# wing02/MyLdpcCppApi

Measured on AMD Instinct MI355X. Metric: decoded Mbit/s (info bits), DVB-S2 N=64800 rate-1/2, 50 iters, higher is better.
Workload: dtype f32; 1 GPU; DVB-S2-profile (64800,32400) rate-1/2 (seeded IRA table with the standard's structure, E=226799), batch 4096 frames per GPU, 50 iterations, sum-product fp32 (probability domain), all-zero codeword + AWGN sigma=0.95 (no frame converges), early termination on, inputs resident in HBM; global_batch=4096, frames_per_gpu=4096, algo=sp, frames_per_launch=4096, parallelism=frames sharded over 1 GPU(s), all-gather of decoded bytes, frames_converged=0

## Files before the change

myldpccppapi_amd/csrc/engine_flood.hip:

```cpp
#include <hip/hip_runtime.h>

#include <algorithm>
#include <map>
#include <vector>

#include "flood_round.hpp"
#include "flood_handover.hpp"
#include "crc_term_kernels.hpp"
#include "decoder.hpp"
#include "graph.hpp"

using ldpc::set_error;

namespace {

using ldpc::DevBuf;
using ldpc::RowClass;
using ldpc::ColClass;
using ldpc::ClassGroup;
using ldpc::kIdleFat;
using ldpc::dispatch_v;
using ldpc::span_begin;
using ldpc::span_end;
using ldpc::kVarBuckets;
using ldpc::kCheckBuckets;
using ldpc::kVarBucketLo;
using ldpc::kVarBucketHi;
using ldpc::kCheckBucketLo;
using ldpc::kCheckBucketHi;

template <int V>
__global__ void summary_kernel(const int32_t *iters, const uint64_t *done, const uint64_t *fail,
                               int64_t frames, int32_t freeze, int32_t *summary)
{
    constexpr int F = 64 * V;
    const int64_t f = (int64_t)blockIdx.x * blockDim.x + threadIdx.x;
    if (f >= frames) return;
    const int64_t tile = f / F;
    const int fi = (int)(f % F);
    const int l = fi / V, v = fi % V;
    atomicMax(&summary[0], iters[f]);
    const uint64_t ok = freeze ? done[tile * V + v] : ~fail[tile * V + v];
    if ((ok >> l) & 1ull) atomicAdd(&summary[1], 1);
}

static inline dim3 flood_grid(const ldpc_decoder *d, unsigned blocks, unsigned tiles, int32_t *tiles_first, bool linked = false)
{
    const bool want = d->tune.tiles_first == 1 || (d->tune.tiles_first == 0 && linked);
    *tiles_first = (blocks <= 65535u && want) ? 1 : 0;
    return *tiles_first ? dim3(tiles, blocks) : dim3(blocks, tiles);
}

static ldpc::CheckArgs check_args(const ldpc_decoder *d, const ldpc::TailRef &tr, int rows_per_wave, bool from_chan,
                                  const int32_t *e0 = nullptr, int n_rows = 0, int degree = 0)
{
    ldpc::CheckArgs a{d->flood.Q.p, d->flood.R.p, e0, d->done.p, d->E, n_rows, rows_per_wave, degree, d->ms_scale, tr};
    a.ms_offset = d->ms_offset;
    a.qpos = d->flood.qpos.p;
// ... 1 lines not shown
    return a;
}

template <int V> int run_flooding(ldpc_decoder *d, const float *llr_dev, int64_t frames,
                                  uint8_t *out_dev, int64_t out_bytes, int32_t *iters_dev,
                                  hipStream_t s, int start_round = 1);

template <int V> int enqueue_check_phase(ldpc_decoder *d, hipStream_t s, int tiles, int64_t frames, int it, int max_iter,
                                         bool fat, const ldpc::TailRef &tr)
{
    using namespace ldpc;
    const int64_t msz = d->flood.msg_size;
    const bool from_chan = it == 1 && d->flood.first_round_from_chan;
    for (auto &rc : d->flood.row_classes) {
        if (!rc.linked) continue;
        LDPC_HIP_TRY(span_begin(d, s, 4, rc.degree,
                           (2 * msz * rc.degree * rc.count + msz * 5 * rc.linked + 2 * msz * d->flood.extra_edges) * frames,
                           msz * ((int64_t)rc.degree * rc.count + rc.linked +
                                  ((int64_t)rc.degree * rc.count - 2 * rc.linked) +
                                  (it < max_iter ? 2 * rc.linked : 0) + 2 * d->flood.extra_edges) * frames));
        CheckArgs a = check_args(d, tr, d->flood.link_rpw, false, rc.e0.p, rc.count, rc.degree);
        LinkArgs lk{rc.link_col.p, rc.link_pos.p, d->flood.chan.p, d->flood.Q.p, d->hard.p, d->N,
                    (it < max_iter) ? 1 : 0, d->tm.tap_iter ? 1 : 0, d->flood.extra_e0.p, d->flood.extra_deg.p, d->flood.n_extra, 0,
                    rc.n_big, rc.small_rows};
        const int variant = (d->flood.link_form == 2 && !d->flood.fns.link_half[rc.degree]) ? 1 : d->flood.link_form;
        const int waves = link_chunk_count(d->flood.link_rpw, rc.n_big, rc.small_rows, rc.count) * (variant == 1 ? V : variant == 2 ? V / 2 : 1);
        lk.link_blocks = (waves + kWavesPerBlock - 1) / kWavesPerBlock;
        const dim3 grid = flood_grid(d, lk.link_blocks + (d->flood.n_extra + kWavesPerBlock - 1) / kWavesPerBlock, tiles, &a.tiles_first, true);
        (variant == 2 ? d->flood.fns.link_half : variant == 1 ? (d->flood.link_deep ? d->flood.fns.link_deep : d->flood.fns.link_narrow) : d->flood.fns.link)
            [rc.degree]<<<grid, kBlock, 0, s>>>(a, lk);
        LDPC_HIP_TRY(span_end(d, s));
    }
    for (auto &g : d->flood.check_groups) {
        int64_t edges = 0;
        for (int i : g.members) edges += (int64_t)d->flood.row_classes[i].degree * d->flood.row_classes[i].count;
        LDPC_HIP_TRY(span_begin(d, s, 5, g.hi, 2 * msz * edges * frames, -1, g.lo));
        CheckArgs a = check_args(d, tr, (d->tune.rows_per_wave ? d->tune.rows_per_wave : 2) * (fat ? kIdleFat : 1), from_chan);
        const dim3 grid = flood_grid(d, fat ? g.blocks_fat : g.blocks, tiles, &a.tiles_first);
        d->flood.fns.check_group[g.bucket]<<<grid, kBlock, 0, s>>>(a, fat ? g.table_fat.p : g.table.p, (int)g.members.size());
        LDPC_HIP_TRY(span_end(d, s));
    }
    for (int ci : d->flood.check_solo) {
        RowClass &rc = d->flood.row_classes[ci];
        LDPC_HIP_TRY(span_begin(d, s, 0, rc.degree, 2 * msz * rc.degree * rc.count * frames));
        const int slotk = rc.degree <= d->flood.fns.max_check_unrolled ? rc.degree : 0;
// ... 117 lines not shown
        } else {
            (void)hipGetLastError();
        }
    }
    const int idle_after = (freeze && !resume && !d->tm.tap_iter && d->cfg.poll_interval == 0) ? d->flood.idle_after : 0;
    const bool use_tail = d->flood.tail_enabled && freeze && !resume && !d->tm.tap_iter && tiles >= 4 * d->flood.TO;
    const TailRef tr{use_tail ? d->flood.tail_state.p : nullptr, d->T, d->flood.TO};
    TailArgs ta{};
    if (use_tail) {
        LDPC_HIP_TRY(hipMemsetAsync(d->flood.tail_state.p, 0, 4 * sizeof(int32_t), s));
        LDPC_HIP_TRY(hipMemsetAsync(d->flood.running.p, 0, d->flood.running.n * sizeof(int32_t), s));
        ta = TailArgs{d->flood.tail_state.p, d->flood.tail_map.p, d->flood.running.p, d->done.p, d->iters.p, d->flood.Q.p, d->flood.chan.p, d->hard.p,
                      d->E, frames, d->N, tiles, d->T, d->flood.TO * F, std::min(d->flood.compact_threshold, d->flood.TO * F), 0, max_iter};
    }

    bool q_less = d->cfg.algo == LDPC_ALGO_MS && !resume && !d->tm.tap_iter && max_iter > 1 && d->flood.n_extra == 0;
    for (auto &rc : d->flood.row_classes) if (rc.linked) q_less = false;
    for (int ci : d->flood.check_solo) if (d->flood.row_classes[ci].degree > d->flood.fns.max_check_unrolled) q_less = false;
    d->flood.first_round_from_chan = q_less;
    if (!resume) {
        LDPC_HIP_TRY(span_begin(d, s, 3));
        InitArgs a{llr_dev, d->flood.chan.p, q_less ? nullptr : d->flood.Q.p, d->hard.p, d->col_ptr.p, d->flood.col_qedge.p,
                   d->E, frames, d->N, d->cfg.llr_scale};
        dim3 grid((d->N + kInitCols - 1) / kInitCols, tiles);
        d->flood.fns.init<<<grid, kBlock, 0, s>>>(a);
        StateArgs st{d->done.p, nullptr, d->iters.p, nullptr, frames, 0, max_iter, freeze ? 1 : 0};
        state_kernel<V><<<use_tail ? d->flood.TA : tiles, 64, 0, s>>>(st);
        LDPC_HIP_TRY(span_end(d, s));
    }

    int launched = start_round - 1;
    bool poll_dense = false;
    for (int it = start_round; it <= rounds; ++it) {
        const bool fat = idle_after > 0 && it > idle_after;
        {
            const int rcp = enqueue_check_phase<V>(d, s, tiles, frames, it, max_iter, fat, tr);
            if (rcp) return rcp;
        }
        {
            const int rcv = enqueue_var_phase<V>(d, s, tiles, frames, it, max_iter, fat, tr);
            if (rcv) return rcv;
        }
        launched = it;
        if (freeze || it == rounds) {
            LDPC_HIP_TRY(span_begin(d, s, 3));
            uint64_t *fw = d->failw.p + (size_t)it * slot;
            const int rbk = (d->M + kBlock - 1) / kBlock;
            SyndromeArgs sa{d->row_ptr.p, d->edge_col.p, d->hard.p, fw, d->done.p, d->M, d->N,
                            d->flood.syn_xcd ? tiles : 0, rbk, tr};
            dim3 sgrid = d->flood.syn_xcd ? dim3(8 * rbk * ((tiles + 7) / 8)) : dim3(rbk, tiles);
            syndrome_kernel<V><<<sgrid, kBlock, 0, s>>>(sa);
            if (d->cfg.crc_kind) {
                CrcTermArgs ca{d->hard.p, fw, d->done.p, d->crc_w.p, d->summary.p + 3, d->N, d->cfg.crc_bits, tr};
                crc_term_kernel<V><<<dim3((unsigned)tiles, V), 64 * crc_term_waves(d->cfg.crc_bits), 0, s>>>(ca);
            }
            StateArgs st{d->done.p, fw, d->iters.p, nullptr, frames, it, max_iter, 1, tr, use_tail ? d->flood.running.p : nullptr,
                         d->summary.p + 2};
            const bool poll = freeze && it < rounds && d->cfg.poll_interval > 0 && !d->host.suppress_poll &&
                              ((it % d->cfg.poll_interval) == 0 || poll_dense);
            if (poll) {
                LDPC_HIP_TRY(hipMemsetAsync(d->active.p, 0, sizeof(int32_t), s));
                st.active = d->active.p;
            }
            state_kernel<V><<<tiles, 64, 0, s>>>(st);
// ... 290 lines not shown

template <int V> int time_check_phase(ldpc_decoder *d, float *ms_out)
{
    hipStream_t s = d->stream.s;
    LDPC_HIP_TRY(hipMemsetAsync(d->flood.Q.p, 0, d->flood.Q.n, s));
    LDPC_HIP_TRY(hipMemsetAsync(d->flood.chan.p, 0, d->flood.chan.n, s));
    LDPC_HIP_TRY(hipMemsetAsync(d->done.p, 0, d->done.n * sizeof(uint64_t), s));
    ldpc::Event ev[2];
    LDPC_HIP_TRY(ev[0].create());
    LDPC_HIP_TRY(ev[1].create());
    float best = 1e30f;
    hipError_t err = hipSuccess;
    int rc = LDPC_OK;
    for (int rep = 0; rep < 4 && err == hipSuccess && rc == LDPC_OK; ++rep) {
        err = hipEventRecord(ev[0].e, s);
        rc = enqueue_check_phase<V>(d, s, d->T, (int64_t)d->T * d->F, 1, d->cfg.max_iter, false, ldpc::TailRef{nullptr, 0, 0});
        if (rc == LDPC_OK)
            rc = enqueue_var_phase<V>(d, s, d->T, (int64_t)d->T * d->F, 1, d->cfg.max_iter, false, ldpc::TailRef{nullptr, 0, 0});
        if (err == hipSuccess) err = hipEventRecord(ev[1].e, s);
        if (err == hipSuccess) err = hipEventSynchronize(ev[1].e);
        float ms = 0;
        if (err == hipSuccess) err = hipEventElapsedTime(&ms, ev[0].e, ev[1].e);
        if (err == hipSuccess && rep > 0 && ms < best) best = ms;
    }
    if (rc) return rc;
    if (err != hipSuccess) return set_error(LDPC_ERR_HIP, "placement search: %s", hipGetErrorString(err));
    *ms_out = best;
    return LDPC_OK;
}

template <int V> int placement_search(ldpc_decoder *d, size_t TF)
{
    const size_t bq = TF * (size_t)d->E * d->flood.msg_size, bc = TF * d->N * d->flood.msg_size;
// ... 62 lines not shown
```

myldpccppapi_amd/csrc/flood_check.hpp:

```cpp
#pragma once

#include "flood_common.hpp"

namespace ldpc {

template <int D, int V>
__device__ __forceinline__ void check_sp(const float (&x)[D][V], float (&out)[D][V])
{
#pragma unroll
    for (int v = 0; v < V; ++v) {
        if (D == 1) { out[0][v] = 1.0f; continue; }
        {
            float p = x[1][v];
#pragma unroll
            for (int j = 2; j < D; ++j) p *= x[j][v];
            out[0][v] = p;
        }
        float pre = x[0][v];
#pragma unroll
        for (int k = 1; k < D; ++k) {
            float p = pre;
#pragma unroll
            for (int j = k + 1; j < D; ++j) p *= x[j][v];
            out[k][v] = p;
// ... 70 lines not shown
    const int tile = tile_select<V>(a.tail, a.done, gp.row);
    if (tile < 0) return;
    const int wave = gp.block * kWavesPerBlock + wave_id_in_block();
    const int sub = wave % SUB;
    const int r_begin = (wave / SUB) * a.rows_per_wave;
    const int r_end = min(r_begin + a.rows_per_wave, a.n_rows);
    const unsigned lane_off = (unsigned)sub * 64 * W + (unsigned)lane * W;
    const T *Qu = static_cast<const T *>(a.Q) + (size_t)tile * (size_t)a.E * F;
    T *Rt = static_cast<T *>(a.R) + (size_t)tile * (size_t)a.E * F + lane_off;

    const T *Ct = (ALGO != kAlgoSP && a.first_chan)
                      ? static_cast<const T *>(a.first_chan) + (size_t)tile * (size_t)a.N * F + lane_off : nullptr;
    check_rows<ALGO, D, V, W, T>(Qu, lane_off, Rt, a.cls_e0, r_begin, r_end, Ct, a.edge_col, a.qpos, ms_corr_of(a));
}

template <int ALGO, int V, typename T>
__device__ __forceinline__ void check_row_generic(const T *Qu, unsigned lane_off, T *Rt, int e0, int D,
                                                  const int32_t *__restrict__ qpos, const MsCorr &c)
{
    constexpr size_t F = 64 * V;
    if (ALGO != kAlgoSP) {
        float m1[V], m2[V];
        int idx[V];
        unsigned par[V];
#pragma unroll
        for (int v = 0; v < V; ++v) { m1[v] = 1000.0f; m2[v] = 1000.0f; idx[v] = -1; par[v] = 0; }
        for (int j = 0; j < D; ++j) {
            float xj[V];
            vload<V>(xj, Qu + (size_t)edge_slot(qpos, e0 + j) * F + lane_off);
#pragma unroll
            for (int v = 0; v < V; ++v) {
                const float m = __builtin_fabsf(xj[v]);
                par[v] ^= (xj[v] < 0.0f) ? 1u : 0u;
                if (m < m1[v]) { m2[v] = m1[v]; m1[v] = m; idx[v] = j; }
                else if (m < m2[v]) { m2[v] = m; }
            }
        }
        if (ALGO == kAlgoMSC) {
#pragma unroll
            for (int v = 0; v < V; ++v) { m1[v] = ms_corr<T>(m1[v], c); m2[v] = ms_corr<T>(m2[v], c); }
        }
        for (int k = 0; k < D; ++k) {
            float xk[V], o[V];
            vload<V>(xk, Qu + (size_t)edge_slot(qpos, e0 + k) * F + lane_off);
#pragma unroll
            for (int v = 0; v < V; ++v) {
                const float b = (k == idx[v]) ? m2[v] : m1[v];
                const unsigned sg = par[v] ^ ((xk[v] < 0.0f) ? 1u : 0u);
                o[v] = sg ? -b : b;
            }
            vstore<V>(Rt + (size_t)(e0 + k) * F, o);
        }
        return;
    }
    for (int k = 0; k < D; ++k) {
        float o[V];
        float p[V];
#pragma unroll
        for (int v = 0; v < V; ++v) p[v] = 1.0f;
        for (int j = 0; j < D; ++j) {
            if (j == k) continue;
            float xj[V];
            vload<V>(xj, Qu + (size_t)edge_slot(qpos, e0 + j) * F + lane_off);
#pragma unroll
            for (int v = 0; v < V; ++v) p[v] *= xj[v];
        }
#pragma unroll
        for (int v = 0; v < V; ++v) o[v] = p[v];
        vstore<V>(Rt + (size_t)(e0 + k) * F, o);
    }
}

template <int ALGO, int V, typename T>
__global__ __launch_bounds__(kBlock) void check_kernel_generic(const CheckArgs a)
{
    constexpr size_t F = 64 * V;
    const int lane = threadIdx.x & 63;
    const GridPos gp = grid_pos(a.tiles_first);
// ... 51 lines not shown
```

myldpccppapi_amd/csrc/flood_common.hpp:

```cpp
#pragma once

#include <hip/hip_runtime.h>
#include <stdint.h>

namespace ldpc {

constexpr int kAlgoSP = 0;
constexpr int kAlgoMS = 1;
constexpr int kAlgoMSC = 2;
constexpr int kCompactCapacity = 512;
constexpr int kLastCapacity = 64;
constexpr int kBlock = 256;
constexpr int kWavesPerBlock = 4;
constexpr int kMaxUnrolledDegree = 16;
constexpr int kMaxUnrolledCheckDegreeMS = 32;

#ifndef LDPC_NT_LOAD
#define LDPC_NT_LOAD 1
#endif
#ifndef LDPC_NT_STORE
#define LDPC_NT_STORE 1
#endif
typedef float vf2 __attribute__((ext_vector_type(2)));
typedef float vf4 __attribute__((ext_vector_type(4)));
// ... 117 lines not shown
    const int32_t *__restrict__ qpos = nullptr;
};

template <int D> __device__ __forceinline__ void row_slots(const int32_t *__restrict__ qpos, int e0, int lane, int (&slot)[D])
{
    static_assert(D <= 64, "one lane per edge");
    const int mine = qpos[e0 + (lane < D ? lane : D - 1)];
#pragma unroll
    for (int k = 0; k < D; ++k) slot[k] = __builtin_amdgcn_readlane(mine, k);
}
__device__ __forceinline__ int edge_slot(const int32_t *__restrict__ qpos, int e)
{
    return __builtin_amdgcn_readfirstlane(qpos[e]);
}

struct GridPos { int row, block; };
__device__ __forceinline__ GridPos grid_pos(int tiles_first)
{
    return tiles_first ? GridPos{(int)blockIdx.x, (int)blockIdx.y} : GridPos{(int)blockIdx.y, (int)blockIdx.x};
}

struct MsCorr {
    float scale, offset;
};
template <typename T> __device__ __forceinline__ float ms_corr(float m, const MsCorr &c)
{
    const float r = fmaxf(m - c.offset, 0.0f) * c.scale;
    return sizeof(T) == 2 ? (float)(hf)r : r;
}

// ... 53 lines not shown
```

myldpccppapi_amd/csrc/flood_link.hpp:

```cpp
#pragma once

#include "flood_check.hpp"
#include "flood_var.hpp"

namespace ldpc {

struct LinkArgs {
    const int32_t *__restrict__ link_col;
    const int32_t *__restrict__ link_pos;
    const void *__restrict__ chan;
    void *Qw;
    uint64_t *hard;
    int32_t N;
    int32_t write_q;
    int32_t store_all;
    const int32_t *__restrict__ extra_e0;
    const int32_t *__restrict__ extra_deg;
    int32_t n_extra;
    int32_t link_blocks;
    int32_t n_big, small_rows;
};

__host__ __device__ inline void link_chunk_rows(int c, int rows_per_wave, int n_big, int small_rows, int n_rows,
                                               int *rb, int *re)
{
    int b, e;
    if (c < n_big) { b = c * rows_per_wave; e = b + rows_per_wave; }
    else { b = n_big * rows_per_wave + (c - n_big) * small_rows; e = b + small_rows; }
    *rb = b < n_rows ? b : n_rows;
    *re = e < n_rows ? e : n_rows;
}
__host__ __device__ inline int link_chunk_count(int rows_per_wave, int n_big, int small_rows, int n_rows)
{
    const int rest = n_rows - n_big * rows_per_wave;
    return n_big + (rest > 0 ? (rest + small_rows - 1) / small_rows : 0);
}

template <int ALGO, int V, typename T>
__device__ __forceinline__ void link_extra_rows(const CheckArgs &a, const LinkArgs &g, int tile, int block)
{
    constexpr size_t F = 64 * V;
    const int lane = threadIdx.x & 63;
    const int w = (block - g.link_blocks) * kWavesPerBlock + wave_id_in_block();
    if (w >= g.n_extra) return;
    const T *Qu = static_cast<const T *>(a.Q) + (size_t)tile * (size_t)a.E * F;
    T *Rt = static_cast<T *>(a.R) + (size_t)tile * (size_t)a.E * F + (size_t)lane * V;
    check_row_generic<ALGO, V, T>(Qu, (unsigned)lane * V, Rt, g.extra_e0[w], g.extra_deg[w], a.qpos, ms_corr_of(a));
}

#ifdef LDPC_LINK_WIDE_WAVES
#define LDPC_LINK_WIDE_ATTR __attribute__((amdgpu_waves_per_eu(LDPC_LINK_WIDE_WAVES, LDPC_LINK_WIDE_WAVES)))
#else
#define LDPC_LINK_WIDE_ATTR
#endif
template <int ALGO, int D, int V, typename T>
__global__ __launch_bounds__(kBlock) LDPC_LINK_WIDE_ATTR void check_link_kernel(const CheckArgs a, const LinkArgs g)
{
    constexpr size_t F = 64 * V;
    const int lane = threadIdx.x & 63;
    const GridPos gp = grid_pos(a.tiles_first);
    const int tile = tile_select<V>(a.tail, a.done, gp.row);
    if (tile < 0) return;
    if (gp.block >= g.link_blocks) { link_extra_rows<ALGO, V, T>(a, g, tile, gp.block); return; }
    const int wave = gp.block * kWavesPerBlock + wave_id_in_block();
    int r_begin, r_end;
    link_chunk_rows(wave, a.rows_per_wave, g.n_big, g.small_rows, a.n_rows, &r_begin, &r_end);
    const size_t lane_off = (size_t)lane * V;
    const unsigned lane_q = (unsigned)lane * V;
    const T *Qt = static_cast<const T *>(a.Q) + (size_t)tile * (size_t)a.E * F;
    T *Qwt = static_cast<T *>(g.Qw) + (size_t)tile * (size_t)a.E * F;
    T *Rt = static_cast<T *>(a.R) + (size_t)tile * (size_t)a.E * F + lane_off;
    const T *chan_t = static_cast<const T *>(g.chan) + (size_t)tile * (size_t)g.N * F + lane_off;
    uint64_t *hard_t = g.hard + (size_t)tile * (size_t)g.N * V;
    uint64_t frozen[V];
#pragma unroll
    for (int v = 0; v < V; ++v) frozen[v] = a.done[(size_t)tile * V + v];

    int pend_col = -1, pend_edge = 0, pend_kb = 0;
    float pend_r[V];
#pragma unroll
    for (int v = 0; v < V; ++v) pend_r[v] = 0.0f;

    float x[D][V];
    int qc[D], qn[D];
#pragma unroll
    for (int k = 0; k < D; ++k) qc[k] = qn[k] = 0;
    if (r_begin < r_end) {
        row_slots<D>(a.qpos, a.cls_e0[r_begin], lane, qc);
#pragma unroll
        for (int k = 0; k < D; ++k) vload<V>(x[k], Qt + (size_t)qc[k] * F + lane_q);
    }
    for (int r = r_begin; r < r_end; ++r) {
        const int e0 = a.cls_e0[r];
        const int next_col = (r + 1 < r_end) ? g.link_col[r] : -1;
        const int pos = g.link_pos[r];
        const int ka = next_col >= 0 ? (pos & 255) : -1;
        const int kb = pend_col >= 0 ? pend_kb : -1;
        if (r + 1 < r_end) row_slots<D>(a.qpos, a.cls_e0[r + 1], lane, qn);
        float ch[V];
        uint64_t old_w[V];
        if (pend_col >= 0) {
            vload<V>(ch, chan_t + (size_t)pend_col * F);
#pragma unroll
            for (int v = 0; v < V; ++v) old_w[v] = hard_t[(size_t)pend_col * V + v];
        }
        float out[D][V];
        check_node<ALGO, D, V, T>(x, out, ms_corr_of(a));
        if (r + 1 < r_end) {
#pragma unroll
            for (int k = 0; k < D; ++k) vload<V>(x[k], Qt + (size_t)qn[k] * F + lane_q);
        }
#pragma unroll
        for (int k = 0; k < D; ++k)
            if ((k != ka && k != kb) || g.store_all) vstore<V>(Rt + (size_t)(e0 + k) * F, out[k]);

        if (pend_col >= 0) {
            float rr[2][V], q[2][V];
#pragma unroll
            for (int v = 0; v < V; ++v) {
                rr[0][v] = pend_r[v];
                float t = out[0][v];
#pragma unroll
                for (int k = 1; k < D; ++k) t = (k == kb) ? out[k][v] : t;
                rr[1][v] = t;
            }
// ... 38 lines not shown
            for (int k = 1; k < D; ++k) pend_edge = (k == ka) ? qc[k] : pend_edge;
            pend_kb = (pos >> 8) & 255;
#pragma unroll
            for (int v = 0; v < V; ++v) {
                float t = out[0][v];
#pragma unroll
                for (int k = 1; k < D; ++k) t = (k == ka) ? out[k][v] : t;
                pend_r[v] = t;
            }
        }
#pragma unroll
        for (int k = 0; k < D; ++k) qc[k] = qn[k];
    }
}

template <int ALGO, int D, int V, typename T, int W = 1>
__global__ __launch_bounds__(kBlock) void check_link_narrow_kernel(const CheckArgs a, const LinkArgs g)
{
    constexpr size_t F = 64 * V;
    constexpr int SUBS = V / W;
    constexpr int FB = 64 / SUBS;
    const int lane = threadIdx.x & 63;
    const GridPos gp = grid_pos(a.tiles_first);
    const int tile = tile_select<V>(a.tail, a.done, gp.row);
    if (tile < 0) return;
    if (gp.block >= g.link_blocks) { link_extra_rows<ALGO, V, T>(a, g, tile, gp.block); return; }
    const int wave = gp.block * kWavesPerBlock + wave_id_in_block();
    const int sub = wave % SUBS;
    int r_begin, r_end;
    link_chunk_rows(wave / SUBS, a.rows_per_wave, g.n_big, g.small_rows, a.n_rows, &r_begin, &r_end);
    const size_t lane_off = (size_t)sub * 64 * W + (size_t)lane * W;
    const unsigned lane_q = (unsigned)lane_off;
    const T *Qt = static_cast<const T *>(a.Q) + (size_t)tile * (size_t)a.E * F;
    T *Qwt = static_cast<T *>(g.Qw) + (size_t)tile * (size_t)a.E * F;
    T *Rt = static_cast<T *>(a.R) + (size_t)tile * (size_t)a.E * F + lane_off;
    const T *chan_t = static_cast<const T *>(g.chan) + (size_t)tile * (size_t)g.N * F + lane_off;
    uint8_t *hard_b = reinterpret_cast<uint8_t *>(g.hard + (size_t)tile * (size_t)g.N * V) + (size_t)sub * (FB / 8);
    const uint64_t frozen_field = (a.done[(size_t)tile * V + (lane < V ? lane : 0)] >> (sub * FB)) &
                                  (FB == 64 ? ~0ull : ((1ull << (FB & 63)) - 1ull));

    auto load_field = [&](int col, int word) -> uint64_t {
// ... 1 lines not shown
        if (FB == 64) return *reinterpret_cast<const uint64_t *>(p);
        if (FB == 32) return *reinterpret_cast<const uint32_t *>(p);
        return *reinterpret_cast<const uint16_t *>(p);
    };

    int pend_col = -1, pend_edge = 0, pend_kb = 0;
    float pend_r[W];
#pragma unroll
    for (int w = 0; w < W; ++w) pend_r[w] = 0.0f;
    float x[D][W];
    int qc[D], qn[D];
#pragma unroll
    for (int k = 0; k < D; ++k) qc[k] = qn[k] = 0;
    if (r_begin < r_end) {
        row_slots<D>(a.qpos, a.cls_e0[r_begin], lane, qc);
#pragma unroll
        for (int k = 0; k < D; ++k) vload<W>(x[k], Qt + (size_t)qc[k] * F + lane_q);
    }
    for (int r = r_begin; r < r_end; ++r) {
        const int e0 = a.cls_e0[r];
        const int next_col = (r + 1 < r_end) ? g.link_col[r] : -1;
        const int pos = g.link_pos[r];
        const int ka = next_col >= 0 ? (pos & 255) : -1;
        const int kb = pend_col >= 0 ? pend_kb : -1;
        if (r + 1 < r_end) row_slots<D>(a.qpos, a.cls_e0[r + 1], lane, qn);
        float ch[W];
        uint64_t old_mine[W];
#pragma unroll
        for (int w = 0; w < W; ++w) { ch[w] = 0.0f; old_mine[w] = 0; }
        if (pend_col >= 0) {
            vload<W>(ch, chan_t + (size_t)pend_col * F);
#pragma unroll
            for (int w = 0; w < W; ++w) old_mine[w] = load_field(pend_col, (W * lane + w) % V);
        }
        float out[D][W];
        check_node<ALGO, D, W, T>(x, out, ms_corr_of(a));
        if (r + 1 < r_end) {
#pragma unroll
            for (int k = 0; k < D; ++k) vload<W>(x[k], Qt + (size_t)qn[k] * F + lane_q);
        }
#pragma unroll
        for (int k = 0; k < D; ++k)
            if ((k != ka && k != kb) || g.store_all) vstore<W>(Rt + (size_t)(e0 + k) * F, out[k]);

        if (pend_col >= 0) {
            float rr[2][W], q[2][W];
#pragma unroll
            for (int w = 0; w < W; ++w) {
                rr[0][w] = pend_r[w];
                float t = out[0][w];
#pragma unroll
                for (int k = 1; k < D; ++k) t = (k == kb) ? out[k][w] : t;
                rr[1][w] = t;
            }
// ... 177 lines not shown
```

myldpccppapi_amd/csrc/flood_round.hpp:

```cpp
#pragma once

#include "flood_common.hpp"
#include "ldpc_expf.h"

namespace ldpc {

struct InitArgs {
    const float *__restrict__ llr;
    void *__restrict__ chan;
    void *__restrict__ Q;
    uint64_t *__restrict__ hard;
    const int32_t *__restrict__ col_ptr;
    const int32_t *__restrict__ col_edge;
    int64_t E;
    int64_t frames;
    int32_t N;
    float llr_scale;
};

constexpr int kInitCols = 32;

template <int ALGO, int V, typename T>
__global__ __launch_bounds__(kBlock) void init_kernel(const InitArgs a)
{
// ... 29 lines not shown
            patch[c * LD + f] = y;
        }
    }
    __syncthreads();
    const int lane = threadIdx.x & 63;
    for (int c = threadIdx.x >> 6; c < kInitCols; c += kWavesPerBlock) {
        const int n = n0 + c;
        if (n >= a.N) break;
        float ch[V], q[V];
#pragma unroll
        for (int v = 0; v < V; ++v) {
            const float y = patch[c * LD + lane * V + v];
            if (ALGO == kAlgoSP) {
                const float t = ldpc_expf(a.llr_scale * y);
                ch[v] = t;
                q[v] = t / (1.0f + t) - 1.0f / (1.0f + t);
            } else {
                ch[v] = y;
                q[v] = y;
            }
        }
        vstore<V>(static_cast<T *>(a.chan) + ((size_t)tile * a.N + n) * F + (size_t)lane * V, ch);
        if (a.Q) {
            const int p0 = a.col_ptr[n], deg = a.col_ptr[n + 1] - p0;
            T *Qt = static_cast<T *>(a.Q) + (size_t)tile * (size_t)a.E * F + (size_t)lane * V;
            for (int k0 = 0; k0 < deg; k0 += 64) {
                const int m = min(64, deg - k0);
                const int mine = a.col_edge[p0 + k0 + (lane < m ? lane : m - 1)];
                for (int k = 0; k < m; ++k)
                    vstore<V>(Qt + (size_t)__builtin_amdgcn_readlane(mine, k) * F, q);
            }
        }
        if (lane < V) a.hard[((size_t)tile * a.N + n) * V + lane] = 0;
    }
}

struct SyndromeArgs {
    const int32_t *__restrict__ row_ptr;
    const int32_t *__restrict__ edge_col;
    const uint64_t *__restrict__ hard;
    uint64_t *__restrict__ fail;
    const uint64_t *__restrict__ done;
    int32_t M, N;
    int32_t tiles;
    int32_t row_blocks;
    TailRef tail;
};

template <int V> __global__ __launch_bounds__(kBlock) void syndrome_kernel(const SyndromeArgs a)
{
    int tile, rb;
    if (a.tiles > 0) {
        const int xcd = blockIdx.x & 7, j = blockIdx.x >> 3;
        tile = xcd + 8 * (j / a.row_blocks);
        rb = j % a.row_blocks;
        if (tile >= a.tiles) return;
    } else {
        tile = blockIdx.y;
        rb = blockIdx.x;
    }
    tile = tile_select<V>(a.tail, a.done, tile);
    if (tile < 0) return;
    const int m = rb * kBlock + threadIdx.x;
    const uint64_t *hard_t = a.hard + (size_t)tile * (size_t)a.N * V;
    uint64_t s[V];
#pragma unroll
    for (int v = 0; v < V; ++v) s[v] = 0;
    if (m < a.M) {
        for (int p = a.row_ptr[m]; p < a.row_ptr[m + 1]; ++p) {
            const int c = a.edge_col[p];
#pragma unroll
            for (int v = 0; v < V; ++v) s[v] ^= hard_t[(size_t)c * V + v];
        }
    }
    __shared__ uint64_t part[kWavesPerBlock][V];
#pragma unroll
    for (int v = 0; v < V; ++v) {
        uint64_t x = s[v];
#pragma unroll
        for (int off = 32; off >= 1; off >>= 1) {
            const uint32_t lo = __shfl_xor((uint32_t)x, off);
            const uint32_t hi = __shfl_xor((uint32_t)(x >> 32), off);
            x |= ((uint64_t)hi << 32) | lo;
        }
        if ((threadIdx.x & 63) == 0) part[threadIdx.x >> 6][v] = x;
    }
    __syncthreads();
    if (threadIdx.x < V) {
        uint64_t x = 0;
#pragma unroll
        for (int w = 0; w < kWavesPerBlock; ++w) x |= part[w][threadIdx.x];
        unsigned long long *dst = reinterpret_cast<unsigned long long *>(&a.fail[(size_t)tile * V + threadIdx.x]);
        const uint64_t seen = __hip_atomic_load(dst, __ATOMIC_RELAXED, __HIP_MEMORY_SCOPE_AGENT);
        if (x & ~seen) atomicOr(dst, (unsigned long long)x);
    }
}

struct StateArgs {
    uint64_t *__restrict__ done;
    const uint64_t *__restrict__ fail;
    int32_t *__restrict__ iters;
    int32_t *__restrict__ active;
    int64_t frames;
    int32_t iter;
    int32_t max_iter;
    int32_t freeze;
    TailRef tail;
    int32_t *__restrict__ running;
    int32_t *__restrict__ tile_rounds;
// ... 105 lines not shown
```

myldpccppapi_amd/csrc/flood_tables.hpp:

```cpp
#pragma once

#include "flood_kernels.hpp"

namespace ldpc {

using CheckFn = void (*)(const CheckArgs);
using VarFn = void (*)(const VarArgs);
using LinkFn = void (*)(const CheckArgs, const LinkArgs);
using CheckGroupFn = void (*)(const CheckArgs, const GroupClass *, int);
using VarGroupFn = void (*)(const VarArgs, const GroupClass *, int);
using InitFn = void (*)(const InitArgs);

constexpr int kVarBuckets = 3, kCheckBuckets = 4;
constexpr int kVarBucketLo[kVarBuckets] = {1, 5, 9}, kVarBucketHi[kVarBuckets] = {4, 8, 16};
constexpr int kCheckBucketLo[kCheckBuckets] = {1, 9, 17, 25}, kCheckBucketHi[kCheckBuckets] = {8, 16, 24, 32};

struct FloodFns {
    CheckFn check[kMaxUnrolledCheckDegreeMS + 1] = {};
    CheckFn check_wide[kMaxUnrolledCheckDegreeMS + 1] = {};
    LinkFn link[kMaxUnrolledDegree + 1] = {};
    LinkFn link_narrow[kMaxUnrolledDegree + 1] = {};
    LinkFn link_deep[kMaxUnrolledDegree + 1] = {};
    LinkFn link_half[kMaxUnrolledDegree + 1] = {};
    VarFn var[kMaxUnrolledDegree + 1] = {};
    CheckGroupFn check_group[kCheckBuckets] = {};
    int check_group_width = 1;
    VarGroupFn var_group[kVarBuckets] = {};
    InitFn init = nullptr;
    int max_check_unrolled = kMaxUnrolledDegree;
};

void fill_flood_sp(int V, FloodFns *f);
void fill_flood_ms(int V, FloodFns *f);
void fill_flood_ms16(int V, FloodFns *f);
void fill_flood_msc(int V, FloodFns *f);
void fill_flood_msc16(int V, FloodFns *f);

}
// ... 1 lines not shown
```

myldpccppapi_amd/csrc/flood_tables_impl.hpp:

```cpp
#pragma once

#include "flood_tables.hpp"

namespace ldpc {
namespace tables {

template <int ALGO, int V, typename T, int D> struct FloodTable {
    static void fill(CheckFn *c, CheckFn *cw, VarFn *v)
    {
        c[D] = check_kernel<ALGO, D, V, 1, T>;
        cw[D] = check_kernel<ALGO, D, V, V, T>;
        v[D] = var_kernel<ALGO, D, V, T>;
        FloodTable<ALGO, V, T, D - 1>::fill(c, cw, v);
    }
};
template <int ALGO, int V, typename T> struct FloodTable<ALGO, V, T, 0> {
    static void fill(CheckFn *c, CheckFn *cw, VarFn *v)
    {
        c[0] = cw[0] = check_kernel_generic<ALGO, V, T>;
        v[0] = var_kernel_generic<ALGO, V, T>;
    }
};

template <int ALGO, int V, typename T, int D> struct CheckTableMS {
    static void fill(CheckFn *c, CheckFn *cw)
    {
        c[D] = cw[D] = check_kernel<ALGO, D, V, 1, T>;
        CheckTableMS<ALGO, V, T, D - 1>::fill(c, cw);
    }
};
template <int ALGO, int V, typename T> struct CheckTableMS<ALGO, V, T, kMaxUnrolledDegree> {
    static void fill(CheckFn *, CheckFn *) {}
};

template <int ALGO, int V, typename T, int D> struct LinkHalf {
    static LinkFn get() { return nullptr; }
};
template <int ALGO, typename T, int D> struct LinkHalf<ALGO, 4, T, D> {
    static LinkFn get() { return check_link_narrow_kernel<ALGO, D, 4, T, 2>; }
};
template <int ALGO, int V, typename T, int D> struct LinkTable {
    static void fill(LinkFn *t, LinkFn *tn, LinkFn *td, LinkFn *th)
    {
        t[D] = check_link_kernel<ALGO, D, V, T>;
        tn[D] = check_link_narrow_kernel<ALGO, D, V, T>;
        td[D] = check_link_narrow2_kernel<ALGO, D, V, T>;
        th[D] = LinkHalf<ALGO, V, T, D>::get();
        LinkTable<ALGO, V, T, D - 1>::fill(t, tn, td, th);
    }
};
template <int ALGO, int V, typename T> struct LinkTable<ALGO, V, T, 1> {
    static void fill(LinkFn *, LinkFn *, LinkFn *, LinkFn *) {}
};

template <int ALGO, int V, typename T> void fill_v(FloodFns *f)
{
    constexpr int DM = kMaxUnrolledDegree;
    FloodTable<ALGO, V, T, DM>::fill(f->check, f->check_wide, f->var);
    LinkTable<ALGO, V, T, DM>::fill(f->link, f->link_narrow, f->link_deep, f->link_half);
    constexpr int GW = (sizeof(T) == 2 && V == 4) ? 2 : 1;
    f->check_group_width = GW;
    f->check_group[0] = check_group_kernel<ALGO, V, T, 1, 8, GW>;
    f->check_group[1] = check_group_kernel<ALGO, V, T, 9, 16, GW>;
    f->check_group[2] = f->check_group[3] = nullptr;
    f->var_group[0] = var_group_kernel<ALGO, V, T, 1, 4>;
    f->var_group[1] = var_group_kernel<ALGO, V, T, 5, 8>;
    f->var_group[2] = var_group_kernel<ALGO, V, T, 9, 16>;
    f->init = init_kernel<ALGO, V, T>;
    f->max_check_unrolled = DM;
    if (ALGO != kAlgoSP) {
        CheckTableMS<ALGO, V, T, kMaxUnrolledCheckDegreeMS>::fill(f->check, f->check_wide);
        f->check_group[2] = check_group_kernel<ALGO, V, T, 17, 24, GW>;
        f->check_group[3] = check_group_kernel<ALGO, V, T, 25, 32, GW>;
        f->max_check_unrolled = kMaxUnrolledCheckDegreeMS;
// ... 14 lines not shown
```

Measured before the change: 1114 Mbit/s.

## Read channel directly in first SP round, chunk syndrome blocks, wave-reduce summary atomics

For sum-product decoding on linked row classes, the first check round now reads channel values through edge_col and converts them with sp_q0, so the init kernel no longer has to write per-edge Q messages for that round. The syndrome kernel now lets each block loop over several row chunks, sized from the CU count, and exits early once every frame in the tile has failed. The summary kernel first reduces within each wave so that only one atomic per wave is issued. The first-round path adds more kernel instantiations and gather-style channel reads, and the tuning probe now times a middle round instead of the first.

```diff
diff --git a/myldpccppapi_amd/csrc/engine_flood.hip b/myldpccppapi_amd/csrc/engine_flood.hip
--- a/myldpccppapi_amd/csrc/engine_flood.hip
+++ b/myldpccppapi_amd/csrc/engine_flood.hip
@@ -35,13 +35,23 @@
 {
     constexpr int F = 64 * V;
     const int64_t f = (int64_t)blockIdx.x * blockDim.x + threadIdx.x;
-    if (f >= frames) return;
-    const int64_t tile = f / F;
-    const int fi = (int)(f % F);
-    const int l = fi / V, v = fi % V;
-    atomicMax(&summary[0], iters[f]);
-    const uint64_t ok = freeze ? done[tile * V + v] : ~fail[tile * V + v];
-    if ((ok >> l) & 1ull) atomicAdd(&summary[1], 1);
+    int32_t it = 0;
+    bool clean = false;
+    if (f < frames) {
+        const int64_t tile = f / F;
+        const int fi = (int)(f % F);
+        const int l = fi / V, v = fi % V;
+        it = iters[f];
+        const uint64_t ok = freeze ? done[tile * V + v] : ~fail[tile * V + v];
+        clean = (ok >> l) & 1ull;
+    }
+#pragma unroll
+    for (int off = 32; off >= 1; off >>= 1) it = max(it, __shfl_xor(it, off));
+    const int n_clean = __popcll(__ballot(clean));
+    if ((threadIdx.x & 63) == 0) {
+        if (it > 0) atomicMax(&summary[0], it);
+        if (n_clean) atomicAdd(&summary[1], n_clean);
+    }
 }
 
 static inline dim3 flood_grid(const ldpc_decoder *d, unsigned blocks, unsigned tiles, int32_t *tiles_first, bool linked = false)
@@ -73,12 +83,13 @@
     const bool from_chan = it == 1 && d->flood.first_round_from_chan;
     for (auto &rc : d->flood.row_classes) {
         if (!rc.linked) continue;
+        const int64_t in = from_chan ? (int64_t)d->N
+                                     : (int64_t)rc.degree * rc.count + rc.linked + d->flood.extra_edges;
         LDPC_HIP_TRY(span_begin(d, s, 4, rc.degree,
                            (2 * msz * rc.degree * rc.count + msz * 5 * rc.linked + 2 * msz * d->flood.extra_edges) * frames,
-                           msz * ((int64_t)rc.degree * rc.count + rc.linked +
-                                  ((int64_t)rc.degree * rc.count - 2 * rc.linked) +
-                                  (it < max_iter ? 2 * rc.linked : 0) + 2 * d->flood.extra_edges) * frames));
-        CheckArgs a = check_args(d, tr, d->flood.link_rpw, false, rc.e0.p, rc.count, rc.degree);
+                           msz * (in + ((int64_t)rc.degree * rc.count - 2 * rc.linked) +
+                                  (it < max_iter ? 2 * rc.linked : 0) + d->flood.extra_edges) * frames));
+        CheckArgs a = check_args(d, tr, d->flood.link_rpw, from_chan, rc.e0.p, rc.count, rc.degree);
         LinkArgs lk{rc.link_col.p, rc.link_pos.p, d->flood.chan.p, d->flood.Q.p, d->hard.p, d->N,
                     (it < max_iter) ? 1 : 0, d->tm.tap_iter ? 1 : 0, d->flood.extra_e0.p, d->flood.extra_deg.p, d->flood.n_extra, 0,
                     rc.n_big, rc.small_rows};
@@ -86,8 +97,10 @@
         const int waves = link_chunk_count(d->flood.link_rpw, rc.n_big, rc.small_rows, rc.count) * (variant == 1 ? V : variant == 2 ? V / 2 : 1);
         lk.link_blocks = (waves + kWavesPerBlock - 1) / kWavesPerBlock;
         const dim3 grid = flood_grid(d, lk.link_blocks + (d->flood.n_extra + kWavesPerBlock - 1) / kWavesPerBlock, tiles, &a.tiles_first, true);
-        (variant == 2 ? d->flood.fns.link_half : variant == 1 ? (d->flood.link_deep ? d->flood.fns.link_deep : d->flood.fns.link_narrow) : d->flood.fns.link)
-            [rc.degree]<<<grid, kBlock, 0, s>>>(a, lk);
+        const LinkFn *form = variant == 2 ? d->flood.fns.link_half
+                             : variant == 1 ? (d->flood.link_deep ? d->flood.fns.link_deep : d->flood.fns.link_narrow) : d->flood.fns.link;
+        if (from_chan) form = d->flood.fns.link_first[variant];
+        form[rc.degree]<<<grid, kBlock, 0, s>>>(a, lk);
         LDPC_HIP_TRY(span_end(d, s));
     }
     for (auto &g : d->flood.check_groups) {
@@ -235,9 +248,25 @@
                       d->E, frames, d->N, tiles, d->T, d->flood.TO * F, std::min(d->flood.compact_threshold, d->flood.TO * F), 0, max_iter};
     }
 
-    bool q_less = d->cfg.algo == LDPC_ALGO_MS && !resume && !d->tm.tap_iter && max_iter > 1 && d->flood.n_extra == 0;
-    for (auto &rc : d->flood.row_classes) if (rc.linked) q_less = false;
-    for (int ci : d->flood.check_solo) if (d->flood.row_classes[ci].degree > d->flood.fns.max_check_unrolled) q_less = false;
+    bool q_less = !resume && !d->tm.tap_iter && max_iter > 1;
+    if (d->cfg.algo == LDPC_ALGO_MS) {
+        q_less = q_less && d->flood.n_extra == 0;
+        for (auto &rc : d->flood.row_classes) if (rc.linked) q_less = false;
+        for (int ci : d->flood.check_solo) if (d->flood.row_classes[ci].degree > d->flood.fns.max_check_unrolled) q_less = false;
+    } else if (d->cfg.algo == LDPC_ALGO_SP) {
+        const int variant = d->flood.link_form;
+        bool linked = false;
+        q_less = q_less && !d->flood.link_deep && d->flood.check_groups.empty() && d->flood.check_solo.empty();
+        for (auto &rc : d->flood.row_classes) {
+            if (!rc.linked) continue;
+            linked = true;
+            const int v = (variant == 2 && !d->flood.fns.link_half[rc.degree]) ? 1 : variant;
+            if (!d->flood.fns.link_first[v][rc.degree]) q_less = false;
+        }
+        q_less = q_less && linked;
+    } else {
+        q_less = false;
+    }
     d->flood.first_round_from_chan = q_less;
     if (!resume) {
         LDPC_HIP_TRY(span_begin(d, s, 3));
@@ -266,9 +295,11 @@
         if (freeze || it == rounds) {
             LDPC_HIP_TRY(span_begin(d, s, 3));
             uint64_t *fw = d->failw.p + (size_t)it * slot;
-            const int rbk = (d->M + kBlock - 1) / kBlock;
+            const int chunks = (d->M + kBlock - 1) / kBlock;
+            const int per = syndrome_chunks_per_block(chunks, tiles, d->flood.cus);
+            const int rbk = (chunks + per - 1) / per;
             SyndromeArgs sa{d->row_ptr.p, d->edge_col.p, d->hard.p, fw, d->done.p, d->M, d->N,
-                            d->flood.syn_xcd ? tiles : 0, rbk, tr};
+                            d->flood.syn_xcd ? tiles : 0, rbk, tr, chunks};
             dim3 sgrid = d->flood.syn_xcd ? dim3(8 * rbk * ((tiles + 7) / 8)) : dim3(rbk, tiles);
             syndrome_kernel<V><<<sgrid, kBlock, 0, s>>>(sa);
             if (d->cfg.crc_kind) {
@@ -589,9 +620,9 @@
     int rc = LDPC_OK;
     for (int rep = 0; rep < 4 && err == hipSuccess && rc == LDPC_OK; ++rep) {
         err = hipEventRecord(ev[0].e, s);
-        rc = enqueue_check_phase<V>(d, s, d->T, (int64_t)d->T * d->F, 1, d->cfg.max_iter, false, ldpc::TailRef{nullptr, 0, 0});
+        rc = enqueue_check_phase<V>(d, s, d->T, (int64_t)d->T * d->F, 2, 3, false, ldpc::TailRef{nullptr, 0, 0});
         if (rc == LDPC_OK)
-            rc = enqueue_var_phase<V>(d, s, d->T, (int64_t)d->T * d->F, 1, d->cfg.max_iter, false, ldpc::TailRef{nullptr, 0, 0});
+            rc = enqueue_var_phase<V>(d, s, d->T, (int64_t)d->T * d->F, 2, 3, false, ldpc::TailRef{nullptr, 0, 0});
         if (err == hipSuccess) err = hipEventRecord(ev[1].e, s);
         if (err == hipSuccess) err = hipEventSynchronize(ev[1].e);
         float ms = 0;
diff --git a/myldpccppapi_amd/csrc/flood_check.hpp b/myldpccppapi_amd/csrc/flood_check.hpp
--- a/myldpccppapi_amd/csrc/flood_check.hpp
+++ b/myldpccppapi_amd/csrc/flood_check.hpp
@@ -108,11 +108,16 @@
     check_rows<ALGO, D, V, W, T>(Qu, lane_off, Rt, a.cls_e0, r_begin, r_end, Ct, a.edge_col, a.qpos, ms_corr_of(a));
 }
 
-template <int ALGO, int V, typename T>
+template <int ALGO, int V, typename T, bool FC = false>
 __device__ __forceinline__ void check_row_generic(const T *Qu, unsigned lane_off, T *Rt, int e0, int D,
-                                                  const int32_t *__restrict__ qpos, const MsCorr &c)
-{
-    constexpr size_t F = 64 * V;
+                                                  const int32_t *__restrict__ qpos, const MsCorr &c,
+                                                  const T *Ct = nullptr, const int32_t *__restrict__ edge_col = nullptr)
+{
+    constexpr size_t F = 64 * V;
+    auto load = [&](float (&x)[V], int e) {
+        if constexpr (FC) first_round_q<ALGO, V, T>(x, Ct + (size_t)__builtin_amdgcn_readfirstlane(edge_col[e]) * F);
+        else vload<V>(x, Qu + (size_t)edge_slot(qpos, e) * F + lane_off);
+    };
     if (ALGO != kAlgoSP) {
         float m1[V], m2[V];
         int idx[V];
@@ -121,7 +126,7 @@
         for (int v = 0; v < V; ++v) { m1[v] = 1000.0f; m2[v] = 1000.0f; idx[v] = -1; par[v] = 0; }
         for (int j = 0; j < D; ++j) {
             float xj[V];
-            vload<V>(xj, Qu + (size_t)edge_slot(qpos, e0 + j) * F + lane_off);
+            load(xj, e0 + j);
 #pragma unroll
             for (int v = 0; v < V; ++v) {
                 const float m = __builtin_fabsf(xj[v]);
@@ -136,7 +141,7 @@
         }
         for (int k = 0; k < D; ++k) {
             float xk[V], o[V];
-            vload<V>(xk, Qu + (size_t)edge_slot(qpos, e0 + k) * F + lane_off);
+            load(xk, e0 + k);
 #pragma unroll
             for (int v = 0; v < V; ++v) {
                 const float b = (k == idx[v]) ? m2[v] : m1[v];
@@ -155,7 +160,7 @@
         for (int j = 0; j < D; ++j) {
             if (j == k) continue;
             float xj[V];
-            vload<V>(xj, Qu + (size_t)edge_slot(qpos, e0 + j) * F + lane_off);
+            load(xj, e0 + j);
 #pragma unroll
             for (int v = 0; v < V; ++v) p[v] *= xj[v];
         }
diff --git a/myldpccppapi_amd/csrc/flood_common.hpp b/myldpccppapi_amd/csrc/flood_common.hpp
--- a/myldpccppapi_amd/csrc/flood_common.hpp
+++ b/myldpccppapi_amd/csrc/flood_common.hpp
@@ -155,6 +155,20 @@
     return __builtin_amdgcn_readfirstlane(qpos[e]);
 }
 
+__device__ __forceinline__ float sp_q0(float t)
+{
+    return t / (1.0f + t) - 1.0f / (1.0f + t);
+}
+
+template <int ALGO, int W, typename T> __device__ __forceinline__ void first_round_q(float (&x)[W], const T *p)
+{
+    vload<W>(x, p);
+    if (ALGO == kAlgoSP) {
+#pragma unroll
+        for (int w = 0; w < W; ++w) x[w] = sp_q0(x[w]);
+    }
+}
+
 struct GridPos { int row, block; };
 __device__ __forceinline__ GridPos grid_pos(int tiles_first)
 {
diff --git a/myldpccppapi_amd/csrc/flood_link.hpp b/myldpccppapi_amd/csrc/flood_link.hpp
--- a/myldpccppapi_amd/csrc/flood_link.hpp
+++ b/myldpccppapi_amd/csrc/flood_link.hpp
@@ -36,7 +36,7 @@
     return n_big + (rest > 0 ? (rest + small_rows - 1) / small_rows : 0);
 }
 
-template <int ALGO, int V, typename T>
+template <int ALGO, int V, typename T, bool FC = false>
 __device__ __forceinline__ void link_extra_rows(const CheckArgs &a, const LinkArgs &g, int tile, int block)
 {
     constexpr size_t F = 64 * V;
@@ -45,7 +45,12 @@
     if (w >= g.n_extra) return;
     const T *Qu = static_cast<const T *>(a.Q) + (size_t)tile * (size_t)a.E * F;
     T *Rt = static_cast<T *>(a.R) + (size_t)tile * (size_t)a.E * F + (size_t)lane * V;
-    check_row_generic<ALGO, V, T>(Qu, (unsigned)lane * V, Rt, g.extra_e0[w], g.extra_deg[w], a.qpos, ms_corr_of(a));
+    if constexpr (FC) {
+        const T *Ct = static_cast<const T *>(g.chan) + (size_t)tile * (size_t)g.N * F + (size_t)lane * V;
+        check_row_generic<ALGO, V, T, true>(Qu, (unsigned)lane * V, Rt, g.extra_e0[w], g.extra_deg[w], a.qpos, ms_corr_of(a), Ct, a.edge_col);
+    } else {
+        check_row_generic<ALGO, V, T>(Qu, (unsigned)lane * V, Rt, g.extra_e0[w], g.extra_deg[w], a.qpos, ms_corr_of(a));
+    }
 }
 
 #ifdef LDPC_LINK_WIDE_WAVES
@@ -53,7 +58,7 @@
 #else
 #define LDPC_LINK_WIDE_ATTR
 #endif
-template <int ALGO, int D, int V, typename T>
+template <int ALGO, int D, int V, typename T, bool FC = false>
 __global__ __launch_bounds__(kBlock) LDPC_LINK_WIDE_ATTR void check_link_kernel(const CheckArgs a, const LinkArgs g)
 {
     constexpr size_t F = 64 * V;
@@ -61,7 +66,7 @@
     const GridPos gp = grid_pos(a.tiles_first);
     const int tile = tile_select<V>(a.tail, a.done, gp.row);
     if (tile < 0) return;
-    if (gp.block >= g.link_blocks) { link_extra_rows<ALGO, V, T>(a, g, tile, gp.block); return; }
+    if (gp.block >= g.link_blocks) { link_extra_rows<ALGO, V, T, FC>(a, g, tile, gp.block); return; }
     const int wave = gp.block * kWavesPerBlock + wave_id_in_block();
     int r_begin, r_end;
     link_chunk_rows(wave, a.rows_per_wave, g.n_big, g.small_rows, a.n_rows, &r_begin, &r_end);
@@ -87,8 +92,15 @@
     for (int k = 0; k < D; ++k) qc[k] = qn[k] = 0;
     if (r_begin < r_end) {
         row_slots<D>(a.qpos, a.cls_e0[r_begin], lane, qc);
-#pragma unroll
-        for (int k = 0; k < D; ++k) vload<V>(x[k], Qt + (size_t)qc[k] * F + lane_q);
+        if constexpr (FC) {
+            int col[D];
+            row_slots<D>(a.edge_col, a.cls_e0[r_begin], lane, col);
+#pragma unroll
+            for (int k = 0; k < D; ++k) first_round_q<ALGO, V, T>(x[k], chan_t + (size_t)col[k] * F);
+        } else {
+#pragma unroll
+            for (int k = 0; k < D; ++k) vload<V>(x[k], Qt + (size_t)qc[k] * F + lane_q);
+        }
     }
     for (int r = r_begin; r < r_end; ++r) {
         const int e0 = a.cls_e0[r];
@@ -107,8 +119,15 @@
         float out[D][V];
         check_node<ALGO, D, V, T>(x, out, ms_corr_of(a));
         if (r + 1 < r_end) {
-#pragma unroll
-            for (int k = 0; k < D; ++k) vload<V>(x[k], Qt + (size_t)qn[k] * F + lane_q);
+            if constexpr (FC) {
+                int col[D];
+                row_slots<D>(a.edge_col, a.cls_e0[r + 1], lane, col);
+#pragma unroll
+                for (int k = 0; k < D; ++k) first_round_q<ALGO, V, T>(x[k], chan_t + (size_t)col[k] * F);
+            } else {
+#pragma unroll
+                for (int k = 0; k < D; ++k) vload<V>(x[k], Qt + (size_t)qn[k] * F + lane_q);
+            }
         }
 #pragma unroll
         for (int k = 0; k < D; ++k)
@@ -177,7 +196,7 @@
     }
 }
 
-template <int ALGO, int D, int V, typename T, int W = 1>
+template <int ALGO, int D, int V, typename T, int W = 1, bool FC = false>
 __global__ __launch_bounds__(kBlock) void check_link_narrow_kernel(const CheckArgs a, const LinkArgs g)
 {
     constexpr size_t F = 64 * V;
@@ -187,7 +206,7 @@
     const GridPos gp = grid_pos(a.tiles_first);
     const int tile = tile_select<V>(a.tail, a.done, gp.row);
     if (tile < 0) return;
-    if (gp.block >= g.link_blocks) { link_extra_rows<ALGO, V, T>(a, g, tile, gp.block); return; }
+    if (gp.block >= g.link_blocks) { link_extra_rows<ALGO, V, T, FC>(a, g, tile, gp.block); return; }
     const int wave = gp.block * kWavesPerBlock + wave_id_in_block();
     const int sub = wave % SUBS;
     int r_begin, r_end;
@@ -219,8 +238,15 @@
     for (int k = 0; k < D; ++k) qc[k] = qn[k] = 0;
     if (r_begin < r_end) {
         row_slots<D>(a.qpos, a.cls_e0[r_begin], lane, qc);
-#pragma unroll
-        for (int k = 0; k < D; ++k) vload<W>(x[k], Qt + (size_t)qc[k] * F + lane_q);
+        if constexpr (FC) {
+            int col[D];
+            row_slots<D>(a.edge_col, a.cls_e0[r_begin], lane, col);
+#pragma unroll
+            for (int k = 0; k < D; ++k) first_round_q<ALGO, W, T>(x[k], chan_t + (size_t)col[k] * F);
+        } else {
+#pragma unroll
+            for (int k = 0; k < D; ++k) vload<W>(x[k], Qt + (size_t)qc[k] * F + lane_q);
+        }
     }
     for (int r = r_begin; r < r_end; ++r) {
         const int e0 = a.cls_e0[r];
@@ -241,8 +267,15 @@
         float out[D][W];
         check_node<ALGO, D, W, T>(x, out, ms_corr_of(a));
         if (r + 1 < r_end) {
-#pragma unroll
-            for (int k = 0; k < D; ++k) vload<W>(x[k], Qt + (size_t)qn[k] * F + lane_q);
+            if constexpr (FC) {
+                int col[D];
+                row_slots<D>(a.edge_col, a.cls_e0[r + 1], lane, col);
+#pragma unroll
+                for (int k = 0; k < D; ++k) first_round_q<ALGO, W, T>(x[k], chan_t + (size_t)col[k] * F);
+            } else {
+#pragma unroll
+                for (int k = 0; k < D; ++k) vload<W>(x[k], Qt + (size_t)qn[k] * F + lane_q);
+            }
         }
 #pragma unroll
         for (int k = 0; k < D; ++k)
diff --git a/myldpccppapi_amd/csrc/flood_round.hpp b/myldpccppapi_amd/csrc/flood_round.hpp
--- a/myldpccppapi_amd/csrc/flood_round.hpp
+++ b/myldpccppapi_amd/csrc/flood_round.hpp
@@ -67,7 +67,7 @@
             if (ALGO == kAlgoSP) {
                 const float t = ldpc_expf(a.llr_scale * y);
                 ch[v] = t;
-                q[v] = t / (1.0f + t) - 1.0f / (1.0f + t);
+                q[v] = sp_q0(t);
             } else {
                 ch[v] = y;
                 q[v] = y;
@@ -98,54 +98,90 @@
     int32_t tiles;
     int32_t row_blocks;
     TailRef tail;
+    int32_t row_chunks;
 };
 
+#ifndef LDPC_SYN_FILL
+#define LDPC_SYN_FILL 2
+#endif
+#ifndef LDPC_SYN_MAX_CHUNKS
+#define LDPC_SYN_MAX_CHUNKS 8
+#endif
+constexpr int kSyndromeFill = LDPC_SYN_FILL, kSyndromeMaxChunks = LDPC_SYN_MAX_CHUNKS;
+
+inline int syndrome_chunks_per_block(int row_chunks, int tiles, int cus)
+{
+    const int slots = kSyndromeFill * (cus > 0 ? cus : 1);
+    const int fill = (int)(((int64_t)row_chunks * tiles + slots - 1) / slots);
+    return fill < 1 ? 1 : (fill > kSyndromeMaxChunks ? kSyndromeMaxChunks : fill);
+}
+
 template <int V> __global__ __launch_bounds__(kBlock) void syndrome_kernel(const SyndromeArgs a)
 {
-    int tile, rb;
+    int tile, rb, nb;
     if (a.tiles > 0) {
         const int xcd = blockIdx.x & 7, j = blockIdx.x >> 3;
         tile = xcd + 8 * (j / a.row_blocks);
         rb = j % a.row_blocks;
+        nb = a.row_blocks;
         if (tile >= a.tiles) return;
     } else {
         tile = blockIdx.y;
         rb = blockIdx.x;
+        nb = gridDim.x;
     }
     tile = tile_select<V>(a.tail, a.done, tile);
     if (tile < 0) return;
-    const int m = rb * kBlock + threadIdx.x;
+    const int chunks = a.row_chunks > 0 ? a.row_chunks : nb;
     const uint64_t *hard_t = a.hard + (size_t)tile * (size_t)a.N * V;
-    uint64_t s[V];
-#pragma unroll
-    for (int v = 0; v < V; ++v) s[v] = 0;
-    if (m < a.M) {
-        for (int p = a.row_ptr[m]; p < a.row_ptr[m + 1]; ++p) {
-            const int c = a.edge_col[p];
-#pragma unroll
-            for (int v = 0; v < V; ++v) s[v] ^= hard_t[(size_t)c * V + v];
-        }
-    }
     __shared__ uint64_t part[kWavesPerBlock][V];
-#pragma unroll
-    for (int v = 0; v < V; ++v) {
-        uint64_t x = s[v];
-#pragma unroll
-        for (int off = 32; off >= 1; off >>= 1) {
-            const uint32_t lo = __shfl_xor((uint32_t)x, off);
-            const uint32_t hi = __shfl_xor((uint32_t)(x >> 32), off);
-            x |= ((uint64_t)hi << 32) | lo;
-        }
-        if ((threadIdx.x & 63) == 0) part[threadIdx.x >> 6][v] = x;
-    }
-    __syncthreads();
+    __shared__ uint64_t open_w[V];
+    unsigned long long *dst = nullptr;
+    uint64_t running = 0;
     if (threadIdx.x < V) {
-        uint64_t x = 0;
-#pragma unroll
-        for (int w = 0; w < kWavesPerBlock; ++w) x |= part[w][threadIdx.x];
-        unsigned long long *dst = reinterpret_cast<unsigned long long *>(&a.fail[(size_t)tile * V + threadIdx.x]);
-        const uint64_t seen = __hip_atomic_load(dst, __ATOMIC_RELAXED, __HIP_MEMORY_SCOPE_AGENT);
-        if (x & ~seen) atomicOr(dst, (unsigned long long)x);
+        dst = reinterpret_cast<unsigned long long *>(&a.fail[(size_t)tile * V + threadIdx.x]);
+        running = ~a.done[(size_t)tile * V + threadIdx.x];
+    }
+    for (int c = rb; c < chunks; c += nb) {
+        if (c != rb) {
+            uint64_t open = 0;
+#pragma unroll
+            for (int v = 0; v < V; ++v) open |= open_w[v];
+            if (!open) return;
+        }
+        const int m = c * kBlock + threadIdx.x;
+        uint64_t s[V];
+#pragma unroll
+        for (int v = 0; v < V; ++v) s[v] = 0;
+        if (m < a.M) {
+            for (int p = a.row_ptr[m]; p < a.row_ptr[m + 1]; ++p) {
+                const int col = a.edge_col[p];
+#pragma unroll
+                for (int v = 0; v < V; ++v) s[v] ^= hard_t[(size_t)col * V + v];
+            }
+        }
+#pragma unroll
+        for (int v = 0; v < V; ++v) {
+            uint64_t x = s[v];
+#pragma unroll
+            for (int off = 32; off >= 1; off >>= 1) {
+                const uint32_t lo = __shfl_xor((uint32_t)x, off);
+                const uint32_t hi = __shfl_xor((uint32_t)(x >> 32), off);
+                x |= ((uint64_t)hi << 32) | lo;
+            }
+            if ((threadIdx.x & 63) == 0) part[threadIdx.x >> 6][v] = x;
+        }
+        __syncthreads();
+        const bool more = c + nb < chunks;
+        if (threadIdx.x < V) {
+            uint64_t x = 0;
+#pragma unroll
+            for (int w = 0; w < kWavesPerBlock; ++w) x |= part[w][threadIdx.x];
+            uint64_t seen = __hip_atomic_load(dst, __ATOMIC_RELAXED, __HIP_MEMORY_SCOPE_AGENT);
+            if (x & ~seen) seen = atomicOr(dst, (unsigned long long)x);
+            if (more) open_w[threadIdx.x] = running & ~(seen | x);
+        }
+        if (more) __syncthreads();
     }
 }
 
diff --git a/myldpccppapi_amd/csrc/flood_tables.hpp b/myldpccppapi_amd/csrc/flood_tables.hpp
--- a/myldpccppapi_amd/csrc/flood_tables.hpp
+++ b/myldpccppapi_amd/csrc/flood_tables.hpp
@@ -22,6 +22,7 @@
     LinkFn link_narrow[kMaxUnrolledDegree + 1] = {};
     LinkFn link_deep[kMaxUnrolledDegree + 1] = {};
     LinkFn link_half[kMaxUnrolledDegree + 1] = {};
+    LinkFn link_first[3][kMaxUnrolledDegree + 1] = {};
     VarFn var[kMaxUnrolledDegree + 1] = {};
     CheckGroupFn check_group[kCheckBuckets] = {};
     int check_group_width = 1;
diff --git a/myldpccppapi_amd/csrc/flood_tables_impl.hpp b/myldpccppapi_amd/csrc/flood_tables_impl.hpp
--- a/myldpccppapi_amd/csrc/flood_tables_impl.hpp
+++ b/myldpccppapi_amd/csrc/flood_tables_impl.hpp
@@ -33,31 +33,36 @@
     static void fill(CheckFn *, CheckFn *) {}
 };
 
-template <int ALGO, int V, typename T, int D> struct LinkHalf {
+template <int ALGO, int V, typename T, int D, bool FC = false> struct LinkHalf {
     static LinkFn get() { return nullptr; }
 };
-template <int ALGO, typename T, int D> struct LinkHalf<ALGO, 4, T, D> {
-    static LinkFn get() { return check_link_narrow_kernel<ALGO, D, 4, T, 2>; }
+template <int ALGO, typename T, int D, bool FC> struct LinkHalf<ALGO, 4, T, D, FC> {
+    static LinkFn get() { return check_link_narrow_kernel<ALGO, D, 4, T, 2, FC>; }
 };
 template <int ALGO, int V, typename T, int D> struct LinkTable {
-    static void fill(LinkFn *t, LinkFn *tn, LinkFn *td, LinkFn *th)
+    static void fill(LinkFn *t, LinkFn *tn, LinkFn *td, LinkFn *th, LinkFn (*first)[kMaxUnrolledDegree + 1])
     {
         t[D] = check_link_kernel<ALGO, D, V, T>;
         tn[D] = check_link_narrow_kernel<ALGO, D, V, T>;
         td[D] = check_link_narrow2_kernel<ALGO, D, V, T>;
         th[D] = LinkHalf<ALGO, V, T, D>::get();
-        LinkTable<ALGO, V, T, D - 1>::fill(t, tn, td, th);
+        if constexpr (ALGO == kAlgoSP) {
+            first[0][D] = check_link_kernel<ALGO, D, V, T, true>;
+            first[1][D] = check_link_narrow_kernel<ALGO, D, V, T, 1, true>;
+            first[2][D] = LinkHalf<ALGO, V, T, D, true>::get();
+        }
+        LinkTable<ALGO, V, T, D - 1>::fill(t, tn, td, th, first);
     }
 };
 template <int ALGO, int V, typename T> struct LinkTable<ALGO, V, T, 1> {
-    static void fill(LinkFn *, LinkFn *, LinkFn *, LinkFn *) {}
+    static void fill(LinkFn *, LinkFn *, LinkFn *, LinkFn *, LinkFn (*)[kMaxUnrolledDegree + 1]) {}
 };
 
 template <int ALGO, int V, typename T> void fill_v(FloodFns *f)
 {
     constexpr int DM = kMaxUnrolledDegree;
     FloodTable<ALGO, V, T, DM>::fill(f->check, f->check_wide, f->var);
-    LinkTable<ALGO, V, T, DM>::fill(f->link, f->link_narrow, f->link_deep, f->link_half);
+    LinkTable<ALGO, V, T, DM>::fill(f->link, f->link_narrow, f->link_deep, f->link_half, f->link_first);
     constexpr int GW = (sizeof(T) == 2 && V == 4) ? 2 : 1;
     f->check_group_width = GW;
     f->check_group[0] = check_group_kernel<ALGO, V, T, 1, 8, GW>;
```

New measurement: 1121 Mbit/s (median of 6 runs). Within noise of the previous version (+0.6%).
